# vshiv18/khoice

Hardware: AMD Instinct MI355X
Metric: distinct k-mers/sec (k=31, canonical) (higher is better)
Workload: dtype u64

## Files before the change

### khoice_amd/csrc/kh_engine.cpp

```cpp
#include <hip/hip_runtime.h>

#include <algorithm>
#include <atomic>
#include <thread>
#include <chrono>
#include <cmath>
#include <memory>
#include <cstdarg>
#include <cstdio>
#include <cstdlib>
#include <cstring>
#include <map>
#include <mutex>
#include <string>
#include <vector>

#include "../../include/khoice_hip.h"
#include "kh_engine.h"
#include "kh_launch.h"
#include "kh_skm_rec.h"

static thread_local std::string g_last_error;

int kh_fail(int code, const char* fmt, ...) {
// ... 1876 lines not shown
        g.m = 16;
        while (g.m >= 14 && !wd.supports_w((u32)(k - g.m + 1))) --g.m;
        if (g.m < 14) return false;
        g.w = (u32)(k - g.m + 1);
        g.nmax = (u32)std::min(63, 118 - k);
    }
    if (!positions) return false;
    g.positions = positions;
    const double clump = skm_clump(g.w, fan);
    const double T = table ? (double)table : (double)wd.table;
    const double r = 0.5 * (-2.5 * std::sqrt(clump) + std::sqrt(6.25 * clump + 4.0 * T));
    u32 mean = (u32)std::max(256.0, r * r);
    if (const char* e = getenv("KHOICE_SKM_MEAN")) mean = std::max<u32>(64, (u32)strtoul(e, nullptr, 10));
    const double per_kmer = skm_per_kmer(g.w);
    double slack1 = 1.25, slack2 = 1.7;
    const u32 max_cap2 = wd.max_cap2;
    for (int it = 0; it < 8; ++it) {
        slack2 = skm_region_slack(clump, (double)mean);
        const double c2 = (double)mean * per_kmer * slack2 + 96 + 16;
        if (c2 <= (double)max_cap2 || mean <= 256) break;
        mean = std::max<u32>(256, (u32)((double)mean * (double)max_cap2 / c2 * 0.98));
    }
    u64 nslots64 = force_slots ? force_slots : std::max<u64>(1, (positions + mean - 1) / mean);
    bool fuller = false;
    const u64 lim = (u64)wd.max_coarse * wd.max_fine;
    if (!force_slots && nslots64 > lim) {
        const double per_slot = (double)positions * per_kmer / (double)lim;
        const double s2 = ((double)max_cap2 - 112.0) / per_slot;
        if (s2 >= 1.4 && (!g.two || (double)positions / (double)lim <= 0.75 * (double)wd.table)) {
            nslots64 = lim;
            slack2 = std::min(slack2, s2);
        }
    }
    const u32 max_coarse = nslots64 > lim ? kh_skm_width(true).max_coarse : wd.max_coarse;
    if (nslots64 > (u64)max_coarse * wd.max_fine) {
        if (!table || force_slots) return false;
        nslots64 = (u64)max_coarse * wd.max_fine;
        fuller = true;
    }
    g.nslots = (u32)nslots64;
    g.S = std::max<u32>(1, (g.nslots + max_coarse - 1) / max_coarse);
    g.nb1 = (g.nslots + g.S - 1) / g.S;
    const double recs = (double)positions * per_kmer;
    if (const char* e = getenv("KHOICE_SKM_SLACK")) slack1 = slack2 = std::max(0.01, atof(e));
    const u64 cap1_64 = ((u64)(recs / g.nb1 * slack1) + 2048 + 63) & ~63ull;
    u64 cap2_64 = ((u64)(recs / g.nslots * slack2) + 96 + 15) & ~15ull;
    if (cap2_64 > max_cap2 && !force_slots && !fuller) {
        if ((double)fan + recs / (double)g.nslots <= (double)max_cap2 - 112.0) cap2_64 = max_cap2 & ~15u;
    }
    if (cap2_64 > max_cap2 || cap1_64 > 0x7fffffffull) return false;
    g.cap1 = (u32)cap1_64;
    g.cap2 = (u32)cap2_64;
    g.ugrid = std::min<u32>(g.nslots, wd.union_per_cu * (u32)std::max(1, cus));
    *out = g;
    return true;
}
template <class F> static int timed_launch(kh_ctx* c, int cls, F launch) {
    c->prof_begin(cls);
    launch();
    c->prof_end();
    HIPCHK(hipGetLastError());
    return KH_OK;
}
struct SkmRun {
    kh_ctx* c;
    TagLayout L;
    SkmGeometry g;
// ... 129 lines not shown
    job.inst = s->dev<unsigned long long>(off.inst);
    job.dup = s->dev<unsigned long long>(off.dup);
    job.ginfo = s->dev<const u32>(off.ginfo);
    job.hist = s->dev<unsigned long long>(0);
    job.ctl = s->dev<u32>(off.ctl);
    job.claim = s->dev<u32>(off.claim);
    job.tile_pos = tile_pos;
    job.k = k; job.m = g.m; job.w = g.w; job.nmax = g.nmax;
    job.nslots = g.nslots; job.S = g.S; job.nb1 = g.nb1; job.cap1 = g.cap1; job.cap2 = g.cap2;
    job.nbins = L->nbins; job.abase = L->abase; job.reps = reps; job.nops = by_group ? (u32)ngroups : (u32)nseq;
    job.spill_rec = s->d_spill.as<uint4>();
    job.spill_slot = reinterpret_cast<u32*>(s->d_spill.as<u8>() + (size_t)spill_cap * rec_bytes);
    job.big_list = reinterpret_cast<u32*>(s->d_spill.as<u8>() + (size_t)spill_cap * (rec_bytes + 4));
    job.spill_cap = spill_cap;
    job.big_cap = SkmRun::big_cap;
#ifdef KH_STAMPS
    const u64 nst = std::max<u64>(ntiles, g.nslots);
    TMP_ALLOC(s->d_stamps, c, 128 * nst);
    HIPCHK(hipMemsetAsync(s->d_stamps.b->p, 0, 128 * nst, st));
    kh_debug_set_stamps_skm(s->d_stamps.as<u64>());
#endif
    c->prof_begin(KC_SKM_SCATTER);
    wd.scatter(job, ntiles, st);
    c->prof_end();
#if defined(KH_STAMPS) && defined(KH_STAMPS_WG)
    dump_wg_ends(c, s->d_stamps.b, ntiles, true);
    HIPCHK(hipMemsetAsync(s->d_stamps.b->p, 0, 128 * nst, st));
    kh_debug_set_stamps_skm(nullptr);
#elif defined(KH_STAMPS)
    report_stamps(c, "skm_scatter (second sub-tile: codes / hashes / minima / slots+count / - / append / barrier / -)", s->d_stamps.b, ntiles);
    HIPCHK(hipMemsetAsync(s->d_stamps.b->p, 0, 128 * nst, st));
    kh_debug_set_stamps_skm(nullptr);
#endif
    c->prof_begin(KC_SKM_REGROUP);
    wd.regroup(job, st);
    c->prof_end();
#ifdef KH_STAMPS
    kh_debug_set_stamps_skm(s->d_stamps.as<u64>());
#ifdef KH_STAMPS_WG
    kh_debug_set_stamps_skm2(s->d_stamps.as<u64>());
#endif
#endif
    s->staged = true;
    return KH_OK;
}
static int exp1_skm(kh_ctx* c, const Exp1In& in, uint64_t* within_hist, uint64_t* across_hist, uint64_t* distinct_per_seq,
                    bool* done, bool by_group = false) {
    *done = false;
    SkmRun s(c);
    KHCHK(skm_prepare(c, in.nseq, in.seqs, in.lens, in.on_device, in.group_of, in.ngroups, in.k, by_group, 0, 0, &s));
    if (!s.staged) return KH_OK;
    const TagLayout& L = s.L;
    const SkmGeometry& g = s.g;
    const KhSkmJob& job = s.job;
    hipStream_t st = c->st;
    KHCHK(timed_launch(c, KC_SKM_UNION, [&] { g.wd->unite(job, in.cs, g.ugrid, st); }));
#if defined(KH_STAMPS) && defined(KH_STAMPS_WG)
    dump_wg_ends(c, s.d_stamps.b, g.ugrid);
    kh_debug_set_stamps_skm(nullptr);
    kh_debug_set_stamps_skm2(nullptr);
#elif defined(KH_STAMPS)
    report_stamps(c, "skm_union (scan barrier / owner / expand / insert / barrier / read-out / barrier / flush)", s.d_stamps.b, g.nslots);
    kh_debug_set_stamps_skm(nullptr);
#endif
    if (getenv("KHOICE_SKM_DEBUG")) {
        std::vector<u32> h1(g.nb1), h2(g.nslots);
        HIPCHK(hipMemcpy2DAsync(h1.data(), 4, job.cur1, 4 * (size_t)KH_SKM_CUR1_STRIDE, 4, g.nb1, hipMemcpyDeviceToHost, st));
        HIPCHK(hipMemcpyAsync(h2.data(), job.cur2, 4 * (size_t)g.nslots, hipMemcpyDeviceToHost, st));
        u32 hc[KH_SKM_CTL_WORDS];
// ... 2093 lines not shown
```

### khoice_amd/csrc/kh_skm_device.h

```cpp
#pragma once
#include <hip/hip_runtime.h>

#include <algorithm>
#include <cstdlib>

#include "kh_device.h"
#include "kh_launch.h"
#include "kh_skm_rec.h"

#ifndef KH_TUNE_SKM_FULL_ROUNDS
#define KH_TUNE_SKM_FULL_ROUNDS 4
#endif

namespace {

constexpr u32 SKM_NT = 256;
constexpr u32 SKM_PPT = 32;
constexpr u32 SKM_SUB = SKM_NT * SKM_PPT;
constexpr u32 SKM_CW = (SKM_SUB + KH_HALO) / 16;
constexpr u32 SKM_CAP = KH_SKM_STAGE;
constexpr int SKM_WMIN = 5, SKM_WMAX = 18;
constexpr u32 SKM_RG_NT = 1024;
static_assert(KH_SKM_MAX_FINE == 1u << SkmRec1::FINE_BITS && KH_SKM2_MAX_FINE == 1u << SkmRec2::FINE_BITS, "a fine slot index fills its field");

// ... 20 lines not shown
__device__ __forceinline__ u32 pick32(const u32 (&v)[SKM_PPT], u32 s) {
    const u32 m0 = 0u - (s & 1u), m1 = 0u - ((s >> 1) & 1u), m2 = 0u - ((s >> 2) & 1u), m3 = 0u - ((s >> 3) & 1u),
              m4 = 0u - ((s >> 4) & 1u);
    u32 a[16], b[8], c[4];
#pragma unroll
    for (int i = 0; i < 16; ++i) a[i] = bsel(m0, v[2 * i + 1], v[2 * i]);
#pragma unroll
    for (int i = 0; i < 8; ++i) b[i] = bsel(m1, a[2 * i + 1], a[2 * i]);
#pragma unroll
    for (int i = 0; i < 4; ++i) c[i] = bsel(m2, b[2 * i + 1], b[2 * i]);
    return bsel(m4, bsel(m3, c[3], c[2]), bsel(m3, c[1], c[0]));
}

template <int WW>
__device__ __forceinline__ void window_min(u32 (&cur)[SKM_PPT + WW - 1]) {
    constexpr int L = WW >= 32 ? 32 : (WW >= 16 ? 16 : (WW >= 8 ? 8 : (WW >= 4 ? 4 : (WW >= 2 ? 2 : 1))));
    constexpr int X = (int)SKM_PPT + WW - 1;
#pragma unroll
    for (int s = 1; s < L; s <<= 1) {
#pragma unroll
        for (int i = 0; i < X - (2 * s - 1); ++i) cur[i] = cur[i] < cur[i + s] ? cur[i] : cur[i + s];
    }
    constexpr int D = WW - L;
    if (D) {
#pragma unroll
        for (int j = 0; j < (int)SKM_PPT; ++j) cur[j] = cur[j] < cur[j + D] ? cur[j] : cur[j + D];
    }
}

struct FlushLds {
    uint4* stage;
    u16* sid;
    u32* bcnt;
    u32* bstart;
    u32* gpos;
    u32* wsum;
};
template <u32 CAP, u32 RW = 4> __device__ __forceinline__ FlushLds flush_lds(u8* base, u32 nbk_alloc) {
    FlushLds L;
    L.stage = reinterpret_cast<uint4*>(base);
    L.sid = reinterpret_cast<u16*>(base + (size_t)CAP * 4 * RW);
    L.bcnt = reinterpret_cast<u32*>(base + (size_t)CAP * (4 * RW + 2));
    L.bstart = L.bcnt + nbk_alloc;
    L.gpos = L.bstart + nbk_alloc + 4;
    L.wsum = L.gpos + nbk_alloc;
    return L;
}
template <u32 CAP, u32 RW = 4> constexpr size_t flush_lds_bytes(u32 nbk_alloc) {
    return (size_t)CAP * (4 * RW + 2) + (size_t)(3 * nbk_alloc + 4 + 16) * 4;
}

struct SkmSpill {
    uint4* rec = nullptr;
    u32* slot = nullptr;
    u32* n = nullptr;
    u32 cap = 0;
    u32 first_slot = 0;
};
template <u32 NT, u32 CAP, bool LOCAL, u32 RW = 4>
__device__ __forceinline__ void skm_flush(const FlushLds& L, const u32 n, const u32 nbk, u32* cursors,
                                          uint4* __restrict__ region, const u32 region_cap, u32* __restrict__ ctl,
                                          const SkmSpill sp = SkmSpill()) {
    constexpr u32 CS = LOCAL ? 1u : KH_SKM_CUR1_STRIDE;
    constexpr int RPT = (int)(CAP / NT);
    const u32 tid = threadIdx.x, lane = lane_id(), wid = tid >> 6;
    u32 c0 = 0, c1 = 0;
    const u32 b0 = 2 * tid, b1 = 2 * tid + 1;
    if (b0 < nbk) c0 = L.bcnt[b0];
    if (b1 < nbk) c1 = L.bcnt[b1];
    const u32 incl = wave_scan_add(c0 + c1);
    if (lane == KH_WAVE - 1) L.wsum[wid] = incl;
    if (c0) {
        u32 g;
        if (LOCAL) { g = cursors[b0]; cursors[b0] = g + c0; }
        else g = atomicAdd(&cursors[(size_t)b0 * CS], c0);
        L.gpos[b0] = g;
        if (g + c0 > region_cap && !sp.rec) atomicOr(ctl, KH_ERR_CAPACITY);
    }
    if (c1) {
        u32 g;
        if (LOCAL) { g = cursors[b1]; cursors[b1] = g + c1; }
        else g = atomicAdd(&cursors[(size_t)b1 * CS], c1);
        L.gpos[b1] = g;
        if (g + c1 > region_cap && !sp.rec) atomicOr(ctl, KH_ERR_CAPACITY);
    }
    constexpr int Q = (int)(RW / 4);
    u32 rx[RPT * Q], ry[RPT * Q], rz[RPT * Q], rw[RPT * Q], bk[RPT];
#pragma unroll
    for (int r = 0; r < RPT; ++r) {
        const u32 i = tid + (u32)r * NT;
#pragma unroll
        for (int q = 0; q < Q; ++q) {
            const uint4 v = L.stage[(i < n ? i : 0) * Q + q];
            rx[r * Q + q] = v.x; ry[r * Q + q] = v.y; rz[r * Q + q] = v.z; rw[r * Q + q] = v.w;
        }
        bk[r] = L.sid[i < n ? i : 0];
    }
    __syncthreads();
    if (!LOCAL) SKM_STAMP(12);
    u32 run = incl - (c0 + c1);
    for (u32 w = 0; w < wid; ++w) run += L.wsum[w];
    if (b0 < nbk) { L.bstart[b0] = run; L.bcnt[b0] = 0; }
    if (b1 < nbk) { L.bstart[b1] = run + c0; L.bcnt[b1] = 0; }
    __syncthreads();
#pragma unroll
    for (int r = 0; r < RPT; ++r) {
        const u32 i = tid + (u32)r * NT;
        if (i < n) {
            const u32 at = L.bstart[bk[r]] + atomicAdd(&L.bcnt[bk[r]], 1u);
#pragma unroll
            for (int q = 0; q < Q; ++q) L.stage[at * Q + q] = make_uint4(rx[r * Q + q], ry[r * Q + q], rz[r * Q + q], rw[r * Q + q]);
            L.sid[at] = (u16)bk[r];
        }
    }
    __syncthreads();
    if (!LOCAL) SKM_STAMP(13);
#pragma unroll
    for (int r = 0; r < RPT; ++r) {
        const u32 i = tid + (u32)r * NT;
        if (i < n) {
            const u32 b = L.sid[i];
            const u32 dest = L.gpos[b] + (i - L.bstart[b]);
            if (dest < region_cap) {
#pragma unroll
                for (int q = 0; q < Q; ++q) region[((u64)b * region_cap + dest) * Q + q] = L.stage[i * Q + q];
            } else if (sp.rec) {
                const u32 at = atomicAdd(sp.n, 1u);
                if (at < sp.cap) {
#pragma unroll
                    for (int q = 0; q < Q; ++q) sp.rec[(u64)at * Q + q] = L.stage[i * Q + q];
                    sp.slot[at] = sp.first_slot + b;
                }
            }
        }
    }
    __syncthreads();
    if (b0 < nbk) L.bcnt[b0] = 0;
    if (b1 < nbk) L.bcnt[b1] = 0;
    __syncthreads();
}

struct SkmFetch { uint4 v[3]; u32 left[3]; };
__device__ __forceinline__ void skm_fetch(const u8* __restrict__ sbase, const u64 len, const u64 p0, SkmFetch& f) {
#pragma unroll
    for (u32 r = 0; r < 3; ++r) {
        const u32 w = threadIdx.x + r * SKM_NT;
        f.left[r] = 0;
        f.v[r] = make_uint4(0, 0, 0, 0);
        if (w < SKM_CW) {
            const u64 b0 = p0 + 16ull * w;
            if (b0 < len) {
                const u64 left = len - b0;
                f.left[r] = left >= 16 ? 16u : (u32)left;
                if (left >= 16) {
                    f.v[r] = *reinterpret_cast<const uint4*>(sbase + b0);
                } else {
                    u32 w4[4] = {0, 0, 0, 0};
                    for (u32 i = 0; i < (u32)left; ++i) w4[i >> 2] |= (u32)sbase[b0 + i] << (8 * (i & 3));
                    f.v[r] = make_uint4(w4[0], w4[1], w4[2], w4[3]);
                }
            }
        }
    }
}
__device__ __forceinline__ void skm_store(const SkmFetch& f, u32* code, u16* bad16) {
#pragma unroll
    for (u32 r = 0; r < 3; ++r) {
        const u32 w = threadIdx.x + r * SKM_NT;
        if (w < SKM_CW) {
            u32 codes = 0, bad = 0xffffu;
            if (f.left[r]) {
// ... 108 lines not shown
    __device__ __forceinline__ SkmSlotFeed(const u32 grid_, const u32 nslots_, const u32 first_claimed)
        : grid(grid_), nslots(nslots_), base(first_claimed), stat(blockIdx.x + 2u * grid_), cnext(0), cend(0) {}
    __device__ __forceinline__ bool wants() const { return B && stat >= base && cnext == cend && cend <= nslots; }
    __device__ __forceinline__ void draw(u32* __restrict__ counter, u32* box) const { *box = base + atomicAdd(counter, B); }
    __device__ __forceinline__ u32 take(const u32* box) {
        if (!B || stat < base) {
            const u32 s = stat;
            stat += grid;
            return s;
        }
        if (cnext == cend && cend <= nslots) {
            cnext = (u32)__builtin_amdgcn_readfirstlane((int)*box);
            cend = cnext + B;
        }
        return cnext++;
    }
};

template <class K> void skm_allow_lds(K kern, size_t bytes) {
    (void)hipFuncSetAttribute(reinterpret_cast<const void*>(kern), hipFuncAttributeMaxDynamicSharedMemorySize, (int)bytes);
}

}

constexpr u32 SKM_RG_U4 = 8192;
template <class Rec> constexpr size_t skm_regroup_lds_bytes(u32 S) {
    return flush_lds_bytes<SKM_RG_U4 / Rec::Q, 4 * Rec::Q>((S + 3) & ~3u) + (size_t)((S + 3) & ~3u) * 4 + 64;
}
template <class Rec>
__global__ __launch_bounds__(SKM_RG_NT, 4) void k_skm_regroup(const KhSkmJob jb) {
    extern __shared__ __attribute__((aligned(16))) u8 lds_raw[];
    constexpr u32 Q = Rec::Q, CAP = SKM_RG_U4 / Q, RW = 4 * Q;
    constexpr int RPT = (int)(CAP / SKM_RG_NT);
    const u32 nbk = (jb.S + 3) & ~3u;
    const FlushLds L = flush_lds<CAP, RW>(lds_raw, nbk);
    u32* lcur = reinterpret_cast<u32*>(lds_raw + flush_lds_bytes<CAP, RW>(nbk));
    const u32 tid = threadIdx.x;
    const u32 b = blockIdx.x;
    const u32 have = jb.cur1[(size_t)b * KH_SKM_CUR1_STRIDE];
    const u32 cnt = have < jb.cap1 ? have : jb.cap1;
    const u32 first_slot = b * jb.S;
    const u32 nfine = jb.nslots - first_slot < jb.S ? jb.nslots - first_slot : jb.S;
    for (u32 i = tid; i < nbk; i += SKM_RG_NT) { L.bcnt[i] = 0; lcur[i] = 0; }
    const uint4* __restrict__ src = jb.reg1 + (u64)b * jb.cap1 * Q;
    uint4* __restrict__ dst = jb.reg2 + (u64)first_slot * jb.cap2 * Q;
    uint4 nx[RPT][Q];
#pragma unroll
    for (int r = 0; r < RPT; ++r) {
        const u32 i = tid + (u32)r * SKM_RG_NT;
#pragma unroll
        for (u32 q = 0; q < Q; ++q) nx[r][q] = i < cnt ? src[Q * i + q] : make_uint4(0, 0, 0, 0);
    }
    __syncthreads();
    for (u32 start = 0; start < cnt; start += CAP) {
        const u32 n = cnt - start < CAP ? cnt - start : CAP;
#pragma unroll
        for (int r = 0; r < RPT; ++r) {
            const u32 i = tid + (u32)r * SKM_RG_NT;
            if (i < n) {
                u32 fine = Rec::fine(nx[r][Q - 1].w);
                if (fine >= nfine) { fine = 0; atomicOr(jb.ctl, KH_ERR_ORDER); }
#pragma unroll
                for (u32 q = 0; q < Q; ++q) L.stage[Q * i + q] = nx[r][q];
                L.sid[i] = (u16)fine;
                atomicAdd(&L.bcnt[fine], 1u);
            }
        }
#pragma unroll
        for (int r = 0; r < RPT; ++r) {
            const u32 i = start + CAP + tid + (u32)r * SKM_RG_NT;
#pragma unroll
            for (u32 q = 0; q < Q; ++q) nx[r][q] = i < cnt ? src[Q * i + q] : make_uint4(0, 0, 0, 0);
        }
        __syncthreads();
        SkmSpill sp;
        sp.rec = jb.spill_rec; sp.slot = jb.spill_slot; sp.n = jb.ctl + KH_SKM_CTL_SPILLED; sp.cap = jb.spill_cap; sp.first_slot = first_slot;
        skm_flush<SKM_RG_NT, CAP, true, RW>(L, n, nfine, lcur, dst, jb.cap2, jb.ctl, sp);
    }
    for (u32 i = tid; i < nfine; i += SKM_RG_NT) jb.cur2[first_slot + i] = lcur[i];
}
template <class Rec> void skm_launch_regroup(const KhSkmJob& job, hipStream_t st) {
    const size_t lds = skm_regroup_lds_bytes<Rec>(job.S);
    skm_allow_lds(k_skm_regroup<Rec>, lds);
    hipLaunchKernelGGL(k_skm_regroup<Rec>, dim3(job.nb1), dim3(SKM_RG_NT), lds, st, job);
}

constexpr u32 SKM_BIG_NT = 1024, SKM_BIG_IDX = 4096;
template <class Tr> constexpr u32 skm_walk_round() { return Tr::T - Tr::T / 4; }

template <class Tr, u32 BINW> struct SkmWalkLds {
    static constexpr u32 T = Tr::T, T2 = Tr::T2, KB = Tr::KEY_BYTES, MAXCH = Tr::BATCH << Tr::OB;
    static constexpr u32 KMAIN = 0, TMLO = KMAIN + T * KB, TMHI = TMLO + T * 4, KSECOND = TMHI + T * 4, OMLO = KSECOND + T2 * KB,
                         OMHI = OMLO + T2 * 4, GTAB = OMHI + T2 * 4, SCRATCH = GTAB + 1024, DUPC = SCRATCH + 128, BINS = DUPC + 256,
                         OWNER = BINS + BINW * 4, SIDX = OWNER + MAXCH * 2;
    static constexpr size_t bytes(bool side) { return SIDX + (side ? SKM_BIG_IDX * 4 : 0); }
    static constexpr u32 OMASK_OFF = (OMLO - TMLO) / 4, OKEY_OFF = (KSECOND - KMAIN) / 8;
    u8* kmain;
    u32* tmlo;
    u32* tmhi;
    u8* ksecond;
    u32* omlo;
    u32* omhi;
    uint4* gtab;
    u32* scratch;
    u32* dupc;
    u32* bins;
    u16* owner;
    u32* sidx;
    __device__ __forceinline__ explicit SkmWalkLds(u8* b)
        : kmain(b + KMAIN), tmlo(reinterpret_cast<u32*>(b + TMLO)), tmhi(reinterpret_cast<u32*>(b + TMHI)), ksecond(b + KSECOND),
          omlo(reinterpret_cast<u32*>(b + OMLO)), omhi(reinterpret_cast<u32*>(b + OMHI)), gtab(reinterpret_cast<uint4*>(b + GTAB)),
          scratch(reinterpret_cast<u32*>(b + SCRATCH)), dupc(reinterpret_cast<u32*>(b + DUPC)), bins(reinterpret_cast<u32*>(b + BINS)),
// ... 288 lines not shown
```

### khoice_amd/csrc/kh_skm.hip

```cpp
#include <hip/hip_runtime.h>

#include "kh_device.h"
#include "kh_launch.h"

#ifdef KH_STAMPS
__device__ u64* g_skm_stamps = nullptr;
void kh_debug_set_stamps_skm(u64* p) { (void)hipMemcpyToSymbol(HIP_SYMBOL(g_skm_stamps), &p, sizeof p); }
#define SKM_STAMP(idx)                                                                     \
    do {                                                                                   \
        __builtin_amdgcn_sched_barrier(0);                                                 \
        if (threadIdx.x == 0 && g_skm_stamps)                                              \
            g_skm_stamps[((u64)blockIdx.y * gridDim.x + blockIdx.x) * 16 + (idx)] = __builtin_amdgcn_s_memtime(); \
        __builtin_amdgcn_sched_barrier(0);                                                 \
    } while (0)
#else
#define SKM_STAMP(idx) do {} while (0)
#endif
#if defined(KH_STAMPS) && defined(KH_STAMPS_WG)
#define SKM_USTAMP(idx) do {} while (0)
#define SKM_WGSTAMP(idx)                                                                   \
    do {                                                                                   \
        __builtin_amdgcn_sched_barrier(0);                                                 \
        if (threadIdx.x == 0 && g_skm_stamps) {                                            \
            u64* const sp_ = g_skm_stamps + (u64)blockIdx.x * 16;                          \
// ... 326 lines not shown
    const u32 tc = ~t;
#pragma unroll
    for (int e = 0; e < E; ++e) {
        if (e) {
            fh = __builtin_amdgcn_alignbit(fh, fl, 30) & kc.kmh;
            fl = ((fl << 2) | ((t >> (2 * e)) & 3u)) & kc.kml;
            rl = __builtin_amdgcn_alignbit(rh, rl, 2);
            rh >>= 2;
            if (kc.tsh_high) rh |= ((tc >> (2 * e)) & 3u) << kc.tsh_sub; else rl |= ((tc >> (2 * e)) & 3u) << kc.tsh_sub;
        }
        const bool fwd = fh < rh || (fh == rh && fl < rl);
        f((u32)e, fwd ? fl : rl, fwd ? fh : rh);
    }
}
struct SkmClaim1 {
    unsigned long long* tkey;
    u32 okey_off;
    unsigned long long empty, K;
    __device__ __forceinline__ u32 operator()(const bool second, const u32 S) const {
        const unsigned long long o2 = atomicCAS(tkey + (second ? okey_off : 0u) + S, empty, K);
        return o2 == empty ? SKM_FRESH : (o2 == K ? SKM_SAME_KEY : SKM_OTHER_KEY);
    }
};

#define KH_TUNE_SKM_UNION_COMPACT 0
template <u32 NT, u32 T, int KT>
__global__ __launch_bounds__(NT, 8) void k_skm_union(const KhSkmJob jb, u32 cs, u32 first_claimed) {
    extern __shared__ __attribute__((aligned(16))) u8 lds_raw[];
    using G = SkmUnionGeo<NT, T>;
    constexpr u32 T2 = G::T2, NW = NT / 64;
    constexpr u32 T2SH = 25;
    constexpr int E = (int)SKM_UE;
    constexpr u64 EMPTY = ~0ull;
    u8* p = lds_raw;
    unsigned long long* tkey = reinterpret_cast<unsigned long long*>(p);   p += (size_t)T * 8;
    u32* tmlo = reinterpret_cast<u32*>(p);                                 p += (size_t)T * 4;
    u32* tmhi = reinterpret_cast<u32*>(p);                                 p += (size_t)T * 4;
    unsigned long long* okey = reinterpret_cast<unsigned long long*>(p);   p += (size_t)T2 * 8;
    u32* omlo = reinterpret_cast<u32*>(p);                                 p += (size_t)T2 * 4;
    u32* omhi = reinterpret_cast<u32*>(p);                                 p += (size_t)T2 * 4;
    uint4* gtab = reinterpret_cast<uint4*>(p);                             p += 1024;
    u32* scratch = reinterpret_cast<u32*>(p);                              p += 128;
    u32* dupc = reinterpret_cast<u32*>(p);                                 p += 256;
    u32* hstripe = reinterpret_cast<u32*>(p);                              p += (size_t)SKM_HSTRIPE_WORDS * 4;
    u16* owner = reinterpret_cast<u16*>(p);                                p += (size_t)G::MAXCH * 2;
    u32* rmask = reinterpret_cast<u32*>(p);
    uint4* stage = reinterpret_cast<uint4*>(tkey);
    u32* dd = reinterpret_cast<u32*>(tkey) + T;
    const u32 tid0 = threadIdx.x;
    u32 tid = tid0, lane = lane_id();
    const u32 nbins = jb.nbins, cap2 = jb.cap2, nslots = jb.nslots;
    const int k = KT ? KT : jb.k;
    const u32 sshift = nbins <= 72u ? 2u : (nbins <= 144u ? 1u : 0u), smask = (1u << sshift) - 1u;
    auto clear_keys = [&]() {
        uint4* k4 = reinterpret_cast<uint4*>(tkey);
        for (u32 i = tid; i < T / 2; i += NT) k4[i] = make_uint4(0xffffffffu, 0xffffffffu, 0xffffffffu, 0xffffffffu);
        unsigned long long e0 = EMPTY;
        asm volatile("" : "+v"(e0));
        if (tid < T2) okey[tid] = e0;
    };
    typedef const u32 __attribute__((address_space(4))) * ConstU32;
    const ConstU32 counts = (ConstU32)(unsigned long long)jb.cur2;
    const u32 fit = cap2 < G::MAXREC ? cap2 : G::MAXREC;
    auto count_of = [&](u32 sl) -> u32 {
        const u32 n = sl < nslots ? counts[sl] : 0u;
        return n <= fit ? n : 0u;
    };
    SKM_MARK("init");
    for (u32 i = tid; i < T / 2; i += NT) reinterpret_cast<uint4*>(tmlo)[i] = make_uint4(0u, 0u, 0u, 0u);
    if (tid < T2) { omlo[tid] = 0u; omhi[tid] = 0u; }
    if (tid < (u32)KH_TAG_MAX_OPS) {
        const u32 g = jb.ginfo[tid], g0 = g & 0xffu, gn = (g >> 8) & 0xffu;
        const u64 gm = gn ? (gn >= 64u ? ~0ull : ((1ull << gn) - 1ull)) << g0 : 0ull;
        gtab[tid] = make_uint4((u32)gm, (u32)(gm >> 32), (g >> 16) << sshift, 0u);
        dupc[tid] = 0;
    }
    if (tid < SKM_HSTRIPE_WORDS) hstripe[tid] = 0;
    if (tid == 0) { scratch[0] = 0; scratch[1] = ~0u; }
    const u32 kml = (u32)kh_mask(2 * k), kmh = (u32)(kh_mask(2 * k) >> 32);
    const u32 fsh = 64u - 2u * (u32)k;
    const u32 tsh = 2u * (u32)k - 2u;
    const bool tsh_high = tsh >= 32u;
    const u32 tsh_sub = tsh_high ? tsh - 32u : tsh;
    auto eval_mask = [&](u32 mlo, u32 mhi) -> bool {
        const u32 lsel = lane & smask;
        u32 ng = 0;
        do {
            const u32 first = mlo ? (u32)__builtin_ctz(mlo) : 32u + (u32)__builtin_ctz(mhi);
            const uint4 g = gtab[first];
            u32 c = (u32)__popc(mlo & g.x) + (u32)__popc(mhi & g.y);
            c = c < cs ? c : cs;
            atomicAdd(&hstripe[g.z + (c << sshift) + lsel], 1u);
            const u32 keep_hi = mlo ? ~0u : mhi - 1u;
            mlo &= ~g.x & (mlo - 1u);
            mhi &= ~g.y & keep_hi;
            ++ng;
        } while (mlo | mhi);
        if (ng == 1u) return true;
        atomicAdd(&hstripe[((jb.abase + (ng < cs ? ng : cs)) << sshift) + lsel], 1u);
        return false;
    };
    u32 st_full = 0, st_exp = 0;
    auto read_out = [&](u32 (&made)[SKM_PASSES][E / 2]) __attribute__((always_inline)) {
        u32 ones = 0;
#pragma unroll
        for (u32 pass = 0; pass < SKM_PASSES; ++pass) {
            u32 any = 0;
#pragma unroll
            for (int e = 0; e < E / 2; ++e) any |= made[pass][e];
            if (!__builtin_amdgcn_ballot_w64(any != 0)) continue;
#pragma unroll
            for (int e = 0; e < E; ++e) {
                const u32 f = (made[pass][e >> 1] >> (16 * (e & 1))) & 0xffffu;
                if (f & 0x8000u) {
                    const u32 at = f & 0x3fffu;
                    const bool second = f & 0x4000u;
                    const u32 mlo = atomicExch((second ? omlo : tmlo) + at, 0u);
                    const u32 mhi = atomicExch((second ? omhi : tmhi) + at, 0u);
                    if (eval_mask(mlo, mhi)) ++ones;
                }
            }
        }
        if (__builtin_amdgcn_ballot_w64(ones != 0)) {
            ones = wave_scan_add(ones);
            if (lane == KH_WAVE - 1) atomicAdd(&hstripe[(jb.abase + 1u) << sshift], ones);
        }
        SKM_MARK("readout_done");
    };
    u32 made_d[SKM_PASSES][E / 2];
#pragma unroll
    for (u32 ps = 0; ps < SKM_PASSES; ++ps)
#pragma unroll
        for (int e = 0; e < E / 2; ++e) made_d[ps][e] = 0u;
    auto read_out_deferred = [&]() __attribute__((always_inline)) {
        read_out(made_d);
#pragma unroll
        for (u32 ps = 0; ps < SKM_PASSES; ++ps)
#pragma unroll
            for (int e = 0; e < E / 2; ++e) made_d[ps][e] = 0u;
    };
    SkmSlotFeed feed(gridDim.x, nslots, first_claimed);
    u32 slot = blockIdx.x, slot_next = slot + gridDim.x;
    u32 nrec = count_of(slot);
    u32 nrec_next = count_of(slot_next);
    uint4 rr = tid < nrec ? (jb.reg2 + (u64)slot * cap2)[tid] : make_uint4(0, 0, 0, 0);
    SKM_WGSTAMP(0);
    [[maybe_unused]] u32 walk_seq = 0;
    while (slot < nslots) {
        tid = tid0;
        asm volatile("" : "+v"(tid));
        lane = tid & (KH_WAVE - 1u);
        const uint4* __restrict__ reg = jb.reg2 + (u64)slot * cap2;
        if (!nrec && counts[slot] > fit) {
            if (tid0 == 0) {
                const u32 at = atomicAdd(jb.ctl + KH_SKM_CTL_LISTED, 1u);
                if (at < jb.big_cap) jb.big_list[at] = slot;
            }
        }
        u32 nj = 0;
// ... 90 lines not shown
        if (C > G::MAXCH) {
            if (tid == 0) {
                if (jb.big_list) {
                    const u32 at = atomicAdd(jb.ctl + KH_SKM_CTL_LISTED, 1u);
                    if (at < jb.big_cap) jb.big_list[at] = slot;
                } else atomicOr(jb.ctl, KH_ERR_CAPACITY);
            }
            C = 0;
            N = 0;
        }
        __syncthreads();
        if (tid == 0) scratch[0] = 0;
        SKM_MARK("owner_done");
        SKM_USTAMP(4);
        const u32 R0 = (N + T - 1) / T;
        auto slot_body = [&](auto multi_) __attribute__((always_inline)) {
            constexpr bool MULTI = decltype(multi_)::value;
            const u32 R = MULTI ? R0 : 1u;
            const u32 c0 = tid;
            for (u32 q = 0; q < R; ++q) {
                if (q) { clear_keys(); __syncthreads(); }
                unsigned long long emptyv = EMPTY;
                asm volatile("" : "+v"(emptyv));
                u32 made[SKM_PASSES][E / 2];
#pragma unroll
                for (u32 ps = 0; ps < SKM_PASSES; ++ps)
#pragma unroll
                    for (int e = 0; e < E / 2; ++e) made[ps][e] = 0u;
#pragma unroll
                for (u32 pass = 0; pass < SKM_PASSES; ++pass) {
                    if (pass * NT >= C) break;
                    const u32 c = pass * NT + c0;
                    u64 kreg[E];
                    u32 slot_[E], act = 0, bits = 0, half = 0;
#pragma unroll
                    for (int e = 0; e < E; ++e) { kreg[e] = EMPTY; slot_[e] = 0; }
                    if (c < C) {
                        const u32 o = owner[c], ri = o >> SKM_OB, first = (o & ((1u << SKM_OB) - 1u)) * (u32)E;
                        const uint4 r0 = reg[ri];
                        bits = rmask[ri];
                        half = SkmRec1::half(r0.w);
                        const u32 left = SkmRec1::n(r0.w) - first;
                        const u32 cnt = left < (u32)E ? left : (u32)E;
                        const u64 clo = ((u64)r0.y << 32) | r0.x, chi = ((u64)r0.w << 32) | r0.z;
                        const u32 sh = 2u * first;
                        const u64 lo = sh ? (clo >> sh) | (chi << (64u - sh)) : clo, hi = chi >> sh;
                        const u32 xl = (u32)lo & kml, xh = (u32)(lo >> 32) & kmh;
                        const u64 fw = kh_revpairs64(((u64)xh << 32) | xl) >> fsh;
                        u32 fl = (u32)fw, fh = (u32)(fw >> 32), rl = ~xl & kml, rh = ~xh & kmh;
                        const u32 t = (u32)((lo >> tsh) | (hi << (64u - tsh)));
                        const u32 tc = ~t;
#pragma unroll
                        for (int e = 0; e < E; ++e) {
                            if (e) {
                                fh = __builtin_amdgcn_alignbit(fh, fl, 30) & kmh;
                                fl = ((fl << 2) | ((t >> (2 * e)) & 3u)) & kml;
                                rl = __builtin_amdgcn_alignbit(rh, rl, 2);
                                rh >>= 2;
                                if (tsh_high) rh |= ((tc >> (2 * e)) & 3u) << tsh_sub; else rl |= ((tc >> (2 * e)) & 3u) << tsh_sub;
                            }
                            const bool fwd = fh < rh || (fh == rh && fl < rl);
                            const u32 cl = fwd ? fl : rl, ch = fwd ? fh : rh;
                            const u32 h = key_hash2(cl, ch);
                            kreg[e] = ((u64)ch << 32) | cl;
                            slot_[e] = (u32)(((u64)h * T) >> 32);
                            if (R != 1 && (u32)e < cnt && (((h >> 4) & 0xffffu) * R) >> 16 == q) act |= 1u << e;
                        }
                        if (R == 1) act = (1u << cnt) - 1u;
                    }
                    SKM_MARK("expanded");
                    if (!__builtin_amdgcn_ballot_w64(act != 0)) continue;
                    u32* const mp = half ? tmhi : tmlo;
                    u32 was[E];
#pragma unroll
// ... 3 lines not shown
                        unsigned long long old[E];
#pragma unroll
                        for (int e = 0; e < E; ++e)
                            old[e] = (act & (1u << e)) ? atomicCAS(&tkey[slot_[e]], emptyv, (unsigned long long)kreg[e]) : 0ull;
#pragma unroll
                        for (int e = 0; e < E; ++e) {
                            if (act & (1u << e)) {
                                const bool fresh = old[e] == emptyv;
                                if (fresh || old[e] == kreg[e]) {
                                    was[e] = atomicOr(mp + slot_[e], bits);
                                    act &= ~(1u << e);
                                    if (fresh) mk |= 1u << e;
                                } else {
                                    slot_[e] = (slot_[e] + 1u) & (T - 1u);
                                }
                            }
                        }
                    };
                    u32 f16[E];
                    auto chain_home = [&](const u32 H) __attribute__((always_inline)) -> u32 { return ((H ^ (H >> 15)) * 0x85EBCA77u) >> T2SH; };
                    auto tier_walk = [&](const unsigned long long K, const u32 H, const u32 kbits, const u32 khalf,
                                         u32 S, bool mine) __attribute__((always_inline)) -> u32 {
                        u32 probes = 0;
                        u32* const kmp = khalf ? tmhi : tmlo;
                        u32 level = 1u, where = 0;
                        while (__builtin_amdgcn_ballot_w64(mine)) {
                            if (mine) {
                                unsigned long long* kp = level == 1 ? okey : tkey;
                                const unsigned long long o2 = atomicCAS(&kp[S], emptyv, K);
                                if (o2 == emptyv || o2 == K) {
                                    u32* mp2 = level == 1 ? (khalf ? omhi : omlo) : kmp;
                                    u32 d = atomicOr(mp2 + S, kbits) & kbits;
                                    while (d) { atomicAdd(&dupc[khalf * 32u + (u32)__builtin_ctz(d)], 1u); d &= d - 1u; }
                                    if (o2 == emptyv) where = 0x8000u | (level == 1 ? 0x4000u : 0u) | S;
                                    mine = false;
                                } else {
                                    ++probes;
                                    if (level == 1 && probes >= 8u) {
                                        level = 2; probes = 0;
                                        S = (u32)(((u64)H * T) >> 32) + (u32)KH_TUNE_SKM_FULL_ROUNDS;
                                        S = S & (T - 1u);
                                    } else if (level == 2 && probes >= T) {
                                        atomicOr(jb.ctl, KH_ERR_CAPACITY);
                                        mine = false;
                                    } else {
                                        S = level == 1 ? ((S + 1u) & (T2 - 1u)) : ((S + 1u) & (T - 1u));
                                    }
                                }
                            }
                        }
                        return where;
                    };
                    auto serial_finish = [&]() __attribute__((always_inline)) {
                        while (__builtin_amdgcn_ballot_w64(act != 0)) {
                            const bool have_one = act != 0;
                            const u32 es = have_one ? (u32)__builtin_ctz(act) : 0u;
                            u64 K = 0;
#pragma unroll
                            for (int e = 0; e < E; ++e)
                                if (es == (u32)e) K = kreg[e];
                            const u32 H = key_hash2((u32)K, (u32)(K >> 32));
                            const u32 where = tier_walk((unsigned long long)K, H, bits, half, chain_home(H), have_one);
                            if (have_one) {
                                act &= ~(1u << es);
#pragma unroll
                                for (int e = 0; e < E; ++e)
                                    if (es == (u32)e) f16[e] = where;
                            }
                        }
                    };
                    for (u32 round = 0; round < (u32)KH_TUNE_SKM_FULL_ROUNDS && __builtin_amdgcn_ballot_w64(act != 0); ++round) probe_round();
                    SKM_USTAMP(9);
                    SKM_MARK("rounds_done");
#pragma unroll
                    for (int e = 0; e < E; ++e) f16[e] = (mk >> e) & 1u ? (0x8000u | slot_[e]) : 0u;
                    serial_finish();
                    SKM_MARK("serial_done");
#pragma unroll
                    for (int e = 0; e < E / 2; ++e) made[pass][e] = f16[2 * e] | (f16[2 * e + 1] << 16);
                    {
                        u32 d = 0;
#pragma unroll
                        for (int e = 0; e < E; ++e) d |= was[e] & bits;
                        if (d) {
#pragma unroll
                            for (int e = 0; e < E; ++e) {
                                u32 de = was[e] & bits;
                                while (de) { atomicAdd(&dupc[half * 32u + (u32)__builtin_ctz(de)], 1u); de &= de - 1u; }
                            }
                        }
                    }
                }
                SKM_MARK("insert_done");
                SKM_USTAMP(5);
                if (draw && q == 0 && tid0 == (NW - 1u) * KH_WAVE) feed.draw(jb.claim, scratch + 1);
                __syncthreads();
                SKM_USTAMP(6);
                if (!MULTI) {
#pragma unroll
                    for (u32 ps = 0; ps < SKM_PASSES; ++ps)
#pragma unroll
                        for (int e = 0; e < E / 2; ++e) made_d[ps][e] = made[ps][e];
                } else {
                    read_out(made);
                    SKM_USTAMP(7);
                }
                if (q + 1 < R) __syncthreads();
            }
        };
        if (R0 == 1u) {
            slot_body(std::false_type{});
        } else if (__builtin_expect(R0 != 0u, 0)) {
// ... 510 lines not shown
```

Baseline: 130.6 billion.

## Restructure SKM flush: fold bucket starts into gpos, batch placement atomics, split write-out

```diff
diff --git a/khoice_amd/csrc/kh_engine.cpp b/khoice_amd/csrc/kh_engine.cpp
--- a/khoice_amd/csrc/kh_engine.cpp
+++ b/khoice_amd/csrc/kh_engine.cpp
@@ -1932,7 +1932,8 @@
             slack2 = std::min(slack2, s2);
         }
     }
-    const u32 max_coarse = nslots64 > lim ? kh_skm_width(true).max_coarse : wd.max_coarse;
+    u32 max_coarse = nslots64 > lim ? kh_skm_width(true).max_coarse : wd.max_coarse;
+    if (const char* e = getenv("KHOICE_SKM_COARSE")) max_coarse = std::min<u32>(max_coarse, (u32)std::max(1, atoi(e)));
     if (nslots64 > (u64)max_coarse * wd.max_fine) {
         if (!table || force_slots) return false;
         nslots64 = (u64)max_coarse * wd.max_fine;
@@ -2128,9 +2129,16 @@
     HIPCHK(hipMemsetAsync(s->d_stamps.b->p, 0, 128 * nst, st));
     kh_debug_set_stamps_skm(nullptr);
 #endif
+#if defined(KH_STAMPS) && !defined(KH_STAMPS_WG)
+    kh_debug_set_stamps_skm(s->d_stamps.as<u64>());
+#endif
     c->prof_begin(KC_SKM_REGROUP);
     wd.regroup(job, st);
     c->prof_end();
+#if defined(KH_STAMPS) && !defined(KH_STAMPS_WG)
+    report_stamps(c, "skm_regroup (second round: stage / flush; 12 scan, 14 starts, 13 placement, 2 write-out; 9 .. 8: the workgroup)", s->d_stamps.b, g.nb1);
+    HIPCHK(hipMemsetAsync(s->d_stamps.b->p, 0, 128 * nst, st));
+#endif
 #ifdef KH_STAMPS
     kh_debug_set_stamps_skm(s->d_stamps.as<u64>());
 #ifdef KH_STAMPS_WG
diff --git a/khoice_amd/csrc/kh_skm_device.h b/khoice_amd/csrc/kh_skm_device.h
--- a/khoice_amd/csrc/kh_skm_device.h
+++ b/khoice_amd/csrc/kh_skm_device.h
@@ -76,22 +76,22 @@
     uint4* stage;
     u16* sid;
     u32* bcnt;
-    u32* bstart;
     u32* gpos;
     u32* wsum;
+    u32* spare;
 };
 template <u32 CAP, u32 RW = 4> __device__ __forceinline__ FlushLds flush_lds(u8* base, u32 nbk_alloc) {
     FlushLds L;
     L.stage = reinterpret_cast<uint4*>(base);
     L.sid = reinterpret_cast<u16*>(base + (size_t)CAP * 4 * RW);
     L.bcnt = reinterpret_cast<u32*>(base + (size_t)CAP * (4 * RW + 2));
-    L.bstart = L.bcnt + nbk_alloc;
-    L.gpos = L.bstart + nbk_alloc + 4;
+    L.gpos = L.bcnt + nbk_alloc;
     L.wsum = L.gpos + nbk_alloc;
+    L.spare = L.wsum + 16;
     return L;
 }
 template <u32 CAP, u32 RW = 4> constexpr size_t flush_lds_bytes(u32 nbk_alloc) {
-    return (size_t)CAP * (4 * RW + 2) + (size_t)(3 * nbk_alloc + 4 + 16) * 4;
+    return (size_t)CAP * (4 * RW + 2) + (size_t)(2 * nbk_alloc + 16 + KH_WAVE) * 4;
 }
 
 struct SkmSpill {
@@ -101,86 +101,134 @@
     u32 cap = 0;
     u32 first_slot = 0;
 };
+__device__ __forceinline__ void skm_pin(u32& x) { asm volatile("" : "+v"(x)); }
 template <u32 NT, u32 CAP, bool LOCAL, u32 RW = 4>
 __device__ __forceinline__ void skm_flush(const FlushLds& L, const u32 n, const u32 nbk, u32* cursors,
                                           uint4* __restrict__ region, const u32 region_cap, u32* __restrict__ ctl,
-                                          const SkmSpill sp = SkmSpill()) {
+                                          const SkmSpill sp = SkmSpill(), const bool stamp = true) {
     constexpr u32 CS = LOCAL ? 1u : KH_SKM_CUR1_STRIDE;
-    constexpr int RPT = (int)(CAP / NT);
+    constexpr int RPT = (int)(CAP / NT), NW = (int)(NT / KH_WAVE);
+    constexpr int Q = (int)(RW / 4);
+    static_assert(NW % 4 == 0 && NW <= 16, "the wave sums are read as uint4");
     const u32 tid = threadIdx.x, lane = lane_id(), wid = tid >> 6;
-    u32 c0 = 0, c1 = 0;
-    const u32 b0 = 2 * tid, b1 = 2 * tid + 1;
-    if (b0 < nbk) c0 = L.bcnt[b0];
-    if (b1 < nbk) c1 = L.bcnt[b1];
+    const bool two = !LOCAL && nbk > NT;
+    const u32 b0 = two ? 2 * tid : tid, b1 = two ? 2 * tid + 1 : ~0u;
+    const bool own0 = b0 < nbk, own1 = b1 < nbk;
+    const u32 v0 = L.bcnt[own0 ? b0 : 0], v1 = L.bcnt[own1 ? b1 : 0];
+    const u32 c0 = own0 ? v0 : 0u, c1 = own1 ? v1 : 0u;
     const u32 incl = wave_scan_add(c0 + c1);
     if (lane == KH_WAVE - 1) L.wsum[wid] = incl;
-    if (c0) {
-        u32 g;
-        if (LOCAL) { g = cursors[b0]; cursors[b0] = g + c0; }
-        else g = atomicAdd(&cursors[(size_t)b0 * CS], c0);
-        L.gpos[b0] = g;
-        if (g + c0 > region_cap && !sp.rec) atomicOr(ctl, KH_ERR_CAPACITY);
-    }
-    if (c1) {
-        u32 g;
-        if (LOCAL) { g = cursors[b1]; cursors[b1] = g + c1; }
-        else g = atomicAdd(&cursors[(size_t)b1 * CS], c1);
-        L.gpos[b1] = g;
-        if (g + c1 > region_cap && !sp.rec) atomicOr(ctl, KH_ERR_CAPACITY);
-    }
-    constexpr int Q = (int)(RW / 4);
+    u32 g0 = 0, g1 = 0;
+    if (LOCAL) {
+        g0 = cursors[own0 ? b0 : 0];
+        if (c0) cursors[b0] = g0 + c0;
+    } else {
+        if (c0) g0 = atomicAdd(&cursors[(size_t)b0 * CS], c0);
+        if (c1) g1 = atomicAdd(&cursors[(size_t)b1 * CS], c1);
+    }
     u32 rx[RPT * Q], ry[RPT * Q], rz[RPT * Q], rw[RPT * Q], bk[RPT];
 #pragma unroll
     for (int r = 0; r < RPT; ++r) {
-        const u32 i = tid + (u32)r * NT;
+        const u32 i = tid + (u32)r * NT, ic = i < n ? i : 0;
 #pragma unroll
         for (int q = 0; q < Q; ++q) {
-            const uint4 v = L.stage[(i < n ? i : 0) * Q + q];
+            const uint4 v = L.stage[ic * Q + q];
             rx[r * Q + q] = v.x; ry[r * Q + q] = v.y; rz[r * Q + q] = v.z; rw[r * Q + q] = v.w;
         }
-        bk[r] = L.sid[i < n ? i : 0];
+        bk[r] = L.sid[ic];
     }
     __syncthreads();
-    if (!LOCAL) SKM_STAMP(12);
+    if (stamp) SKM_STAMP(12);
     u32 run = incl - (c0 + c1);
-    for (u32 w = 0; w < wid; ++w) run += L.wsum[w];
-    if (b0 < nbk) { L.bstart[b0] = run; L.bcnt[b0] = 0; }
-    if (b1 < nbk) { L.bstart[b1] = run + c0; L.bcnt[b1] = 0; }
+    {
+        uint4 ws[NW / 4];
+#pragma unroll
+        for (int j = 0; j < NW / 4; ++j) ws[j] = reinterpret_cast<const uint4*>(L.wsum)[j];
+#pragma unroll
+        for (int j = 0; j < NW / 4; ++j) {
+            run += (4u * j + 0 < wid ? ws[j].x : 0u) + (4u * j + 1 < wid ? ws[j].y : 0u) + (4u * j + 2 < wid ? ws[j].z : 0u) +
+                   (4u * j + 3 < wid ? ws[j].w : 0u);
+        }
+    }
+    if (own0) { L.bcnt[b0] = run; L.gpos[b0] = g0 - run; }
+    if (own1) { L.bcnt[b1] = run + c0; L.gpos[b1] = g1 - (run + c0); }
+    if (!sp.rec && ((c0 && g0 + c0 > region_cap) || (c1 && g1 + c1 > region_cap))) atomicOr(ctl, KH_ERR_CAPACITY);
     __syncthreads();
+    if (stamp) SKM_STAMP(14);
+    u32 at[RPT], sl = lane;
+    skm_pin(sl);
 #pragma unroll
     for (int r = 0; r < RPT; ++r) {
-        const u32 i = tid + (u32)r * NT;
-        if (i < n) {
-            const u32 at = L.bstart[bk[r]] + atomicAdd(&L.bcnt[bk[r]], 1u);
-#pragma unroll
-            for (int q = 0; q < Q; ++q) L.stage[at * Q + q] = make_uint4(rx[r * Q + q], ry[r * Q + q], rz[r * Q + q], rw[r * Q + q]);
-            L.sid[at] = (u16)bk[r];
+        const bool live = tid + (u32)r * NT < n;
+        u32* const counter = live ? &L.bcnt[bk[r]] : &L.spare[sl];
+        at[r] = atomicAdd(counter, live ? 1u : 0u);
+    }
+#pragma unroll
+    for (int r = 0; r < RPT; ++r) skm_pin(at[r]);
+#pragma unroll
+    for (int r = 0; r < RPT; ++r) {
+        if (tid + (u32)r * NT < n) {
+#pragma unroll
+            for (int q = 0; q < Q; ++q) L.stage[at[r] * Q + q] = make_uint4(rx[r * Q + q], ry[r * Q + q], rz[r * Q + q], rw[r * Q + q]);
+            L.sid[at[r]] = (u16)bk[r];
         }
     }
     __syncthreads();
-    if (!LOCAL) SKM_STAMP(13);
-#pragma unroll
-    for (int r = 0; r < RPT; ++r) {
-        const u32 i = tid + (u32)r * NT;
-        if (i < n) {
-            const u32 b = L.sid[i];
-            const u32 dest = L.gpos[b] + (i - L.bstart[b]);
-            if (dest < region_cap) {
-#pragma unroll
-                for (int q = 0; q < Q; ++q) region[((u64)b * region_cap + dest) * Q + q] = L.stage[i * Q + q];
-            } else if (sp.rec) {
-                const u32 at = atomicAdd(sp.n, 1u);
-                if (at < sp.cap) {
-#pragma unroll
-                    for (int q = 0; q < Q; ++q) sp.rec[(u64)at * Q + q] = L.stage[i * Q + q];
-                    sp.slot[at] = sp.first_slot + b;
+    if (stamp) SKM_STAMP(13);
+    if (own0) L.bcnt[b0] = 0;
+    if (own1) L.bcnt[b1] = 0;
+    constexpr int G = RPT > 1 ? RPT / 2 : 1;
+    static_assert(RPT % G == 0, "halves of equal size");
+    auto half = [&](const int h) __attribute__((always_inline)) {
+        u32 wb[G], dest[G], vx[G * Q], vy[G * Q], vz[G * Q], vw[G * Q];
+#pragma unroll
+        for (int r = 0; r < G; ++r) {
+            const u32 i = tid + (u32)(h + r) * NT, ic = i < n ? i : 0;
+            wb[r] = L.sid[ic];
+#pragma unroll
+            for (int q = 0; q < Q; ++q) {
+                const uint4 v = L.stage[ic * Q + q];
+                vx[r * Q + q] = v.x; vy[r * Q + q] = v.y; vz[r * Q + q] = v.z; vw[r * Q + q] = v.w;
+            }
+        }
+#pragma unroll
+        for (int r = 0; r < G; ++r) skm_pin(wb[r]);
+#pragma unroll
+        for (int r = 0; r < G; ++r) dest[r] = L.gpos[wb[r]] + tid + (u32)(h + r) * NT;
+        bool over = false;
+#pragma unroll
+        for (int r = 0; r < G; ++r) {
+            skm_pin(dest[r]);
+            if (tid + (u32)(h + r) * NT >= n) dest[r] = 0;
+#pragma unroll
+            for (int q = 0; q < Q; ++q) { skm_pin(vx[r * Q + q]); skm_pin(vy[r * Q + q]); skm_pin(vz[r * Q + q]); skm_pin(vw[r * Q + q]); }
+            over |= dest[r] >= region_cap;
+        }
+#pragma unroll
+        for (int r = 0; r < G; ++r) {
+            if (tid + (u32)(h + r) * NT < n && dest[r] < region_cap) {
+#pragma unroll
+                for (int q = 0; q < Q; ++q)
+                    region[((u64)wb[r] * region_cap + dest[r]) * Q + q] = make_uint4(vx[r * Q + q], vy[r * Q + q], vz[r * Q + q], vw[r * Q + q]);
+            }
+        }
+        if (sp.rec && __ballot(over)) {
+#pragma unroll
+            for (int r = 0; r < G; ++r) {
+                if (tid + (u32)(h + r) * NT < n && dest[r] >= region_cap) {
+                    const u32 slot = atomicAdd(sp.n, 1u);
+                    if (slot < sp.cap) {
+#pragma unroll
+                        for (int q = 0; q < Q; ++q)
+                            sp.rec[(u64)slot * Q + q] = make_uint4(vx[r * Q + q], vy[r * Q + q], vz[r * Q + q], vw[r * Q + q]);
+                        sp.slot[slot] = sp.first_slot + wb[r];
+                    }
                 }
             }
         }
-    }
-    __syncthreads();
-    if (b0 < nbk) L.bcnt[b0] = 0;
-    if (b1 < nbk) L.bcnt[b1] = 0;
+    };
+    half(0);
+    if (RPT > 1) half(G);
     __syncthreads();
 }
 
@@ -355,11 +403,13 @@
     extern __shared__ __attribute__((aligned(16))) u8 lds_raw[];
     constexpr u32 Q = Rec::Q, CAP = SKM_RG_U4 / Q, RW = 4 * Q;
     constexpr int RPT = (int)(CAP / SKM_RG_NT);
+    static_assert(KH_SKM_MAX_FINE <= SKM_RG_NT && KH_SKM2_MAX_FINE <= SKM_RG_NT, "the flush gives every slot of the bucket a thread");
     const u32 nbk = (jb.S + 3) & ~3u;
     const FlushLds L = flush_lds<CAP, RW>(lds_raw, nbk);
     u32* lcur = reinterpret_cast<u32*>(lds_raw + flush_lds_bytes<CAP, RW>(nbk));
     const u32 tid = threadIdx.x;
     const u32 b = blockIdx.x;
+    SKM_STAMP(9);
     const u32 have = jb.cur1[(size_t)b * KH_SKM_CUR1_STRIDE];
     const u32 cnt = have < jb.cap1 ? have : jb.cap1;
     const u32 first_slot = b * jb.S;
@@ -377,6 +427,8 @@
     __syncthreads();
     for (u32 start = 0; start < cnt; start += CAP) {
         const u32 n = cnt - start < CAP ? cnt - start : CAP;
+        const bool stamp = start == CAP;
+        if (stamp) SKM_STAMP(0);
 #pragma unroll
         for (int r = 0; r < RPT; ++r) {
             const u32 i = tid + (u32)r * SKM_RG_NT;
@@ -396,11 +448,14 @@
             for (u32 q = 0; q < Q; ++q) nx[r][q] = i < cnt ? src[Q * i + q] : make_uint4(0, 0, 0, 0);
         }
         __syncthreads();
+        if (stamp) SKM_STAMP(1);
         SkmSpill sp;
         sp.rec = jb.spill_rec; sp.slot = jb.spill_slot; sp.n = jb.ctl + KH_SKM_CTL_SPILLED; sp.cap = jb.spill_cap; sp.first_slot = first_slot;
-        skm_flush<SKM_RG_NT, CAP, true, RW>(L, n, nfine, lcur, dst, jb.cap2, jb.ctl, sp);
+        skm_flush<SKM_RG_NT, CAP, true, RW>(L, n, nfine, lcur, dst, jb.cap2, jb.ctl, sp, stamp);
+        if (stamp) SKM_STAMP(2);
     }
     for (u32 i = tid; i < nfine; i += SKM_RG_NT) jb.cur2[first_slot + i] = lcur[i];
+    SKM_STAMP(8);
 }
 template <class Rec> void skm_launch_regroup(const KhSkmJob& job, hipStream_t st) {
     const size_t lds = skm_regroup_lds_bytes<Rec>(job.S);
```

Result: no change. 131.8 billion, median of 6 (+0.9%).

## Merge primary and overflow tables and carry owner group to skip first lookup

Applied to the files above, without the earlier changes.

```diff
diff --git a/khoice_amd/csrc/kh_skm.hip b/khoice_amd/csrc/kh_skm.hip
--- a/khoice_amd/csrc/kh_skm.hip
+++ b/khoice_amd/csrc/kh_skm.hip
@@ -382,13 +382,17 @@
     constexpr u32 T2SH = 25;
     constexpr int E = (int)SKM_UE;
     constexpr u64 EMPTY = ~0ull;
+    constexpr u32 MADE_FIELD_BITS = 13, MADE_FIELD = (1u << MADE_FIELD_BITS) - 1u, MADE_FIELDS = (1u << (2 * MADE_FIELD_BITS)) - 1u;
+    constexpr u32 MADE_OWN_SHIFT = 2 * MADE_FIELD_BITS;
+    static_assert(T + T2 <= MADE_FIELD, "a field of `made` holds a joint index + 1");
+    static_assert(KH_TAG_MAX_OPS <= (1 << (32 - MADE_OWN_SHIFT)), "a word of `made` holds an operand number above its fields");
     u8* p = lds_raw;
-    unsigned long long* tkey = reinterpret_cast<unsigned long long*>(p);   p += (size_t)T * 8;
-    u32* tmlo = reinterpret_cast<u32*>(p);                                 p += (size_t)T * 4;
-    u32* tmhi = reinterpret_cast<u32*>(p);                                 p += (size_t)T * 4;
-    unsigned long long* okey = reinterpret_cast<unsigned long long*>(p);   p += (size_t)T2 * 8;
-    u32* omlo = reinterpret_cast<u32*>(p);                                 p += (size_t)T2 * 4;
-    u32* omhi = reinterpret_cast<u32*>(p);                                 p += (size_t)T2 * 4;
+    unsigned long long* tkey = reinterpret_cast<unsigned long long*>(p);   p += (size_t)(T + T2) * 8;
+    u32* tmlo = reinterpret_cast<u32*>(p);                                 p += (size_t)(T + T2) * 4;
+    u32* tmhi = reinterpret_cast<u32*>(p);                                 p += (size_t)(T + T2) * 4;
+    unsigned long long* const okey = tkey + T;
+    u32* const omlo = tmlo + T;
+    u32* const omhi = tmhi + T;
     uint4* gtab = reinterpret_cast<uint4*>(p);                             p += 1024;
     u32* scratch = reinterpret_cast<u32*>(p);                              p += 128;
     u32* dupc = reinterpret_cast<u32*>(p);                                 p += 256;
@@ -417,12 +421,11 @@
         return n <= fit ? n : 0u;
     };
     SKM_MARK("init");
-    for (u32 i = tid; i < T / 2; i += NT) reinterpret_cast<uint4*>(tmlo)[i] = make_uint4(0u, 0u, 0u, 0u);
-    if (tid < T2) { omlo[tid] = 0u; omhi[tid] = 0u; }
+    for (u32 i = tid; i < (T + T2) / 2; i += NT) reinterpret_cast<uint4*>(tmlo)[i] = make_uint4(0u, 0u, 0u, 0u);
     if (tid < (u32)KH_TAG_MAX_OPS) {
         const u32 g = jb.ginfo[tid], g0 = g & 0xffu, gn = (g >> 8) & 0xffu;
         const u64 gm = gn ? (gn >= 64u ? ~0ull : ((1ull << gn) - 1ull)) << g0 : 0ull;
-        gtab[tid] = make_uint4((u32)gm, (u32)(gm >> 32), (g >> 16) << sshift, 0u);
+        gtab[tid] = make_uint4((u32)gm, (u32)(gm >> 32), (g >> 16) << (sshift + 2u), 0u);
         dupc[tid] = 0;
     }
     if (tid < SKM_HSTRIPE_WORDS) hstripe[tid] = 0;
@@ -432,22 +435,30 @@
     const u32 tsh = 2u * (u32)k - 2u;
     const bool tsh_high = tsh >= 32u;
     const u32 tsh_sub = tsh_high ? tsh - 32u : tsh;
-    auto eval_mask = [&](u32 mlo, u32 mhi) -> bool {
-        const u32 lsel = lane & smask;
-        u32 ng = 0;
-        do {
-            const u32 first = mlo ? (u32)__builtin_ctz(mlo) : 32u + (u32)__builtin_ctz(mhi);
-            const uint4 g = gtab[first];
-            u32 c = (u32)__popc(mlo & g.x) + (u32)__popc(mhi & g.y);
+    auto eval_mask = [&](u32 mlo, u32 mhi, const uint4 g, const u32 own) -> bool {
+        const u32 bsh = sshift + 2u;
+        u8* const hlane = reinterpret_cast<u8*>(hstripe) + ((lane & smask) << 2);
+        auto count_group = [&](const uint4 gg) {
+            u32 c = (u32)__popc(mlo & gg.x) + (u32)__popc(mhi & gg.y);
             c = c < cs ? c : cs;
-            atomicAdd(&hstripe[g.z + (c << sshift) + lsel], 1u);
+            atomicAdd(reinterpret_cast<u32*>(hlane + (gg.z + (c << bsh))), 1u);
+        };
+        count_group(g);
+        if (!__builtin_amdgcn_ballot_w64(((mlo & ~g.x) | (mhi & ~g.y)) != 0u)) return true;
+        const u32 ob = 1u << (own & 31u);
+        mlo &= ~(g.x | (own < 32u ? ob : 0u));
+        mhi &= ~(g.y | (own < 32u ? 0u : ob));
+        u32 ng = 1;
+        while (mlo | mhi) {
+            const uint4 g2 = gtab[mlo ? (u32)__builtin_ctz(mlo) : 32u + (u32)__builtin_ctz(mhi)];
+            count_group(g2);
             const u32 keep_hi = mlo ? ~0u : mhi - 1u;
-            mlo &= ~g.x & (mlo - 1u);
-            mhi &= ~g.y & keep_hi;
+            mlo &= ~g2.x & (mlo - 1u);
+            mhi &= ~g2.y & keep_hi;
             ++ng;
-        } while (mlo | mhi);
+        }
         if (ng == 1u) return true;
-        atomicAdd(&hstripe[((jb.abase + (ng < cs ? ng : cs)) << sshift) + lsel], 1u);
+        atomicAdd(&hstripe[((jb.abase + (ng < cs ? ng : cs)) << sshift) + (lane & smask)], 1u);
         return false;
     };
     u32 st_full = 0, st_exp = 0;
@@ -457,24 +468,26 @@
         for (u32 pass = 0; pass < SKM_PASSES; ++pass) {
             u32 any = 0;
 #pragma unroll
-            for (int e = 0; e < E / 2; ++e) any |= made[pass][e];
+            for (int e = 0; e < E / 2; ++e) any |= made[pass][e] & MADE_FIELDS;
             if (!__builtin_amdgcn_ballot_w64(any != 0)) continue;
+            const u32 own = made[pass][0] >> MADE_OWN_SHIFT;
+            const uint4 g = gtab[own];
 #pragma unroll
             for (int e = 0; e < E; ++e) {
-                const u32 f = (made[pass][e >> 1] >> (16 * (e & 1))) & 0xffffu;
-                if (f & 0x8000u) {
-                    const u32 at = f & 0x3fffu;
-                    const bool second = f & 0x4000u;
-                    const u32 mlo = atomicExch((second ? omlo : tmlo) + at, 0u);
-                    const u32 mhi = atomicExch((second ? omhi : tmhi) + at, 0u);
-                    if (eval_mask(mlo, mhi)) ++ones;
-                }
-            }
-        }
-        if (__builtin_amdgcn_ballot_w64(ones != 0)) {
-            ones = wave_scan_add(ones);
-            if (lane == KH_WAVE - 1) atomicAdd(&hstripe[(jb.abase + 1u) << sshift], ones);
-        }
+                const u32 f = (made[pass][e >> 1] >> (MADE_FIELD_BITS * (e & 1))) & MADE_FIELD;
+                bool one = false;
+                if (f) {
+                    const u32 mlo = atomicExch(tmlo + f - 1u, 0u);
+                    const u32 mhi = atomicExch(tmhi + f - 1u, 0u);
+                    uint4 ge = g;
+                    u32 owne = own;
+                    asm volatile("" : "+v"(ge.x), "+v"(ge.y), "+v"(ge.z), "+v"(owne));
+                    one = eval_mask(mlo, mhi, ge, owne);
+                }
+                ones += (u32)__builtin_popcountll(__builtin_amdgcn_ballot_w64(one));
+            }
+        }
+        if (ones && lane == 0) atomicAdd(&hstripe[(jb.abase + 1u) << sshift], ones);
         SKM_MARK("readout_done");
     };
     u32 made_d[SKM_PASSES][E / 2];
@@ -631,7 +644,7 @@
                     if (pass * NT >= C) break;
                     const u32 c = pass * NT + c0;
                     u64 kreg[E];
-                    u32 slot_[E], act = 0, bits = 0, half = 0;
+                    u32 slot_[E], act = 0, bits = 0, half = 0, own = 0;
 #pragma unroll
                     for (int e = 0; e < E; ++e) { kreg[e] = EMPTY; slot_[e] = 0; }
                     if (c < C) {
@@ -639,6 +652,7 @@
                         const uint4 r0 = reg[ri];
                         bits = rmask[ri];
                         half = SkmRec1::half(r0.w);
+                        own = SkmRec1::tag(r0.w);
                         const u32 left = SkmRec1::n(r0.w) - first;
                         const u32 cnt = left < (u32)E ? left : (u32)E;
                         const u64 clo = ((u64)r0.y << 32) | r0.x, chi = ((u64)r0.w << 32) | r0.z;
@@ -708,7 +722,7 @@
                                     u32* mp2 = level == 1 ? (khalf ? omhi : omlo) : kmp;
                                     u32 d = atomicOr(mp2 + S, kbits) & kbits;
                                     while (d) { atomicAdd(&dupc[khalf * 32u + (u32)__builtin_ctz(d)], 1u); d &= d - 1u; }
-                                    if (o2 == emptyv) where = 0x8000u | (level == 1 ? 0x4000u : 0u) | S;
+                                    if (o2 == emptyv) where = (level == 1 ? T : 0u) + S + 1u;
                                     mine = false;
                                 } else {
                                     ++probes;
@@ -749,11 +763,11 @@
                     SKM_USTAMP(9);
                     SKM_MARK("rounds_done");
 #pragma unroll
-                    for (int e = 0; e < E; ++e) f16[e] = (mk >> e) & 1u ? (0x8000u | slot_[e]) : 0u;
+                    for (int e = 0; e < E; ++e) f16[e] = (mk >> e) & 1u ? slot_[e] + 1u : 0u;
                     serial_finish();
                     SKM_MARK("serial_done");
 #pragma unroll
-                    for (int e = 0; e < E / 2; ++e) made[pass][e] = f16[2 * e] | (f16[2 * e + 1] << 16);
+                    for (int e = 0; e < E / 2; ++e) made[pass][e] = f16[2 * e] | (f16[2 * e + 1] << MADE_FIELD_BITS) | (own << MADE_OWN_SHIFT);
                     {
                         u32 d = 0;
 #pragma unroll
```

Measured after the change: 130.5 billion before, 132.7 billion after, median of 6. 1.02x the previous value.
